# ZrrSkywalker/MonoDETR

Hardware: NVIDIA H100
Metric: images/sec (1280x384, fwd+bwd) (higher is better)
Workload: dtype f32 (BF16x3: error-compensated bf16 tensor-core products, fp32 accumulate)

## Files before the change

monodetr_b200/csrc/conv_gemm.cu:

```cuda
#include <cuda.h>
#include <cuda_runtime.h>
#include <stdint.h>
#include <stdlib.h>
#include <string.h>

#include "../../include/monodetr_b200.h"
#include "launch.cuh"
#include "tc_common.cuh"
#include "tma_host.cuh"

namespace {

using namespace mdb;

constexpr int BM = 128;
constexpr int BK = 32;
constexpr int kTileABytes = BM * 128;
constexpr int kChunkBytes = 32 * 128;
constexpr int kConsumerThreads = 256;
constexpr int kThreadsTC = kConsumerThreads + 128;
constexpr int kProducerRegs = 40;
constexpr int kConsumerRegs = 232;
constexpr int kMaxTaps = 9;

struct TcParams {
    int tiles_x, tiles_y, tw, th, tb;
    int Ho, Wo;
    int out_sy, out_sx, out_oy, out_ox, out_H, out_W;
    int in_sy, in_sx;
    int ntaps, cblocks;
    int tap_dy[kMaxTaps], tap_dx[kMaxTaps], tap_w[kMaxTaps];
    int rtiles_x, rtiles_y, rtw, rth, n_img, red_per_split;
    int kb_per_slice, slice_stride;
    int total_tiles, n_tiles_n, n_tiles_m;
    int w_sy, w_sx, wg_taps, wg_kw, wg_pad;
    int Mo_rows;
    int No, ldo;
    int relu, atomic_out, round_out;
    int epi_tma, epi_load, half_x, half_y, half_b;
    const float* bias;
    const float* residual;
    const float* relu_mask;
    const float* rowscale;
    float* out;
};

template <bool MN>
__device__ __forceinline__ uint32_t raw_off(int row, int k) {
    if constexpr (MN) return (uint32_t)((row >> 5) * kChunkBytes + k * 128 + (((((row & 31) >> 2) ^ (k & 7))) << 4) + (row & 3) * 4);
    else return (uint32_t)(row * 128 + (((k >> 2) ^ (row & 7)) << 4) + (k & 3) * 4);
}

__device__ __forceinline__ float trunc_tf32(float x) { return __uint_as_float(__float_as_uint(x) & 0xFFFFE000u); }

template <int BN, int STAGES, int MODE, int PREC>
struct TcSmem {
    static constexpr bool kConvB = !(PREC == 2 && MODE == 0);
    static constexpr int kRing = STAGES * (kTileABytes + BN * 128);
    static constexpr int kConvBuf = kConvB ? (PREC == 1 ? 2 : 1) * BN * 128 : 0;
    static constexpr int kConv = 2 * kConvBuf;
    static constexpr int kFixed = kRing + kConv + 1024  + 256 ;
    static constexpr int kChunks = BN / 32;
    static constexpr int kRoom = (227 * 1024 - kFixed) / (2 * 8192);
    static constexpr int kBufs = kRoom >= kChunks ? kChunks : BN < 256 ? 0 : kRoom >= 4 ? 4 : kRoom >= 2 ? 2 : kRoom;
    static constexpr int kStage = 2 * kBufs * 8192;
    static constexpr bool kTmaEpi = MODE == 0 && kBufs > 0;
    static constexpr int kBytes = kFixed + (kTmaEpi ? kStage : 0);
};

template <int BN, int STAGES, int MODE , bool B_MN, int PREC>
__global__ void __launch_bounds__(kThreadsTC, 1)
tc_conv_gemm_kernel(const __grid_constant__ CUtensorMap mapA, const __grid_constant__ CUtensorMap mapB,
                    const __grid_constant__ CUtensorMap mapO, const __grid_constant__ CUtensorMap mapR,
                    const __grid_constant__ TcParams p) {
    constexpr bool A_MN = (MODE == 1);
    static_assert(!(MODE == 1) || B_MN, "wgrad reads both operands MN-major");
    constexpr bool BF_B = (PREC == 2 && MODE == 0);
    static_assert(BN == 64 || BN == 128 || (BN == 256 && BF_B), "tile width");
    static_assert(!BF_B || !B_MN, "pre-split weights are K-major");
    constexpr bool CONVB = !BF_B;
    constexpr int kTileBBytes = BN * 128;
    constexpr int kRawBytes = kTileABytes + kTileBBytes;
    using SM = TcSmem<BN, STAGES, MODE, PREC>;
    constexpr int NACC = BN / 2;

    extern __shared__ __align__(1024) uint8_t smem[];
    uint8_t* stage_out = smem + STAGES * kRawBytes;
    uint8_t* bconv = stage_out + (SM::kTmaEpi ? SM::kStage : 0);
    uint64_t* full_bar = reinterpret_cast<uint64_t*>(bconv + SM::kConv);
    uint64_t* empty_bar = full_bar + STAGES;
    constexpr int kRound = SM::kBufs >= SM::kChunks ? SM::kChunks : 1;
    constexpr int kSlots = SM::kBufs / kRound > 0 ? SM::kBufs / kRound : 1;
    constexpr int kRounds = SM::kChunks / kRound;
    static_assert(kRounds % kSlots == 0, "every slot serves the same number of rounds per tile");
    uint64_t* epi_bar = empty_bar + STAGES;

    const int warp = threadIdx.x >> 5;
    const int lane = threadIdx.x & 31;

    struct Tile { int n0, img, y0, x0, m0, red_begin, iters, tap, slice; };
    auto decode = [&](int tix) {
        Tile t;
        t.n0 = (tix % p.n_tiles_n) * BN;
        int r = tix / p.n_tiles_n;
        t.img = t.y0 = t.x0 = t.m0 = t.red_begin = t.tap = t.slice = 0;
        if constexpr (MODE == 0) {
            const int per_img = p.tiles_x * p.tiles_y;
            t.iters = p.ntaps * p.cblocks;
            if (p.kb_per_slice > 0) {
                t.slice = r / p.n_tiles_m;
                r -= t.slice * p.n_tiles_m;
                t.red_begin = t.slice * p.kb_per_slice;
                t.iters = max(0, min(t.iters, t.red_begin + p.kb_per_slice) - t.red_begin);
            }
            const int grp = r / per_img;
            t.img = grp * p.tb;
            r -= grp * per_img;
            t.y0 = (r / p.tiles_x) * p.th;
            t.x0 = (r % p.tiles_x) * p.tw;
        } else {
            t.m0 = (r % p.n_tiles_m) * BM;
            r /= p.n_tiles_m;
            t.tap = r % p.wg_taps;
            const int z = r / p.wg_taps;
            const int total_red = p.n_img * p.rtiles_x * p.rtiles_y;
            t.red_begin = z * p.red_per_split;
            t.iters = max(0, min(total_red, t.red_begin + p.red_per_split) - t.red_begin);
        }
        return t;
    };

    if (threadIdx.x == 0) {
        if (smem_u32(smem) & 1023u) __trap();
        tma_prefetch_desc(&mapA);
        tma_prefetch_desc(&mapB);
        if (SM::kTmaEpi && p.epi_tma) {
            tma_prefetch_desc(&mapO);
            if (p.epi_load) tma_prefetch_desc(&mapR);
        }
        for (int s = 0; s < STAGES; ++s) {
            mbar_init(&full_bar[s], 1);
            mbar_init(&empty_bar[s], kConsumerThreads / 32);
        }
        for (int i = 0; i < 2 * kSlots; ++i) mbar_init(&epi_bar[i], 1);
        fence_mbar_init();
    }
    __syncthreads();
    asm volatile("griddepcontrol.wait;" ::: "memory");
    asm volatile("griddepcontrol.launch_dependents;" ::: "memory");

    if (warp >= kConsumerThreads / 32) {
        setmaxnreg_dec<kProducerRegs>();
        if (warp == kConsumerThreads / 32 && elect_one()) {
            int git = 0;
            for (int tix = blockIdx.x; tix < p.total_tiles; tix += gridDim.x) {
                const Tile t = decode(tix);
                for (int it = 0; it < t.iters; ++it, ++git) {
                    const int s = git % STAGES;
                    const uint32_t ph = (git / STAGES) & 1;
                    mbar_wait(&empty_bar[s], ph ^ 1);
                    uint8_t* a_dst = smem + s * kRawBytes;
                    uint8_t* b_dst = a_dst + kTileABytes;
                    mbar_arrive_expect_tx(&full_bar[s], kRawBytes);
                    if constexpr (MODE == 0) {
                        const int kit = t.red_begin + it;
                        const int tap = kit / p.cblocks;
                        const int cb = kit - tap * p.cblocks;
                        tma_load_4d(a_dst, &mapA, &full_bar[s], cb * BK, t.x0 * p.in_sx + p.tap_dx[tap],
                                    t.y0 * p.in_sy + p.tap_dy[tap], t.img);
                        if constexpr (BF_B) {
                            tma_load_3d(b_dst, &mapB, &full_bar[s], cb * 64, t.n0, p.tap_w[tap]);
                        } else if constexpr (!B_MN) {
                            tma_load_3d(b_dst, &mapB, &full_bar[s], cb * BK, t.n0, p.tap_w[tap]);
                        } else {
#pragma unroll
                            for (int j = 0; j < BN / 32; ++j)
                                tma_load_3d(b_dst + j * kChunkBytes, &mapB, &full_bar[s], t.n0 + j * 32, cb * BK, p.tap_w[tap]);
                        }
                    } else {
                        int r = t.red_begin + it;
                        const int per_img = p.rtiles_x * p.rtiles_y;
                        const int ri = r / per_img;
                        r -= ri * per_img;
                        const int ry = (r / p.rtiles_x) * p.rth;
                        const int rx = (r % p.rtiles_x) * p.rtw;
#pragma unroll
                        for (int j = 0; j < BM / 32; ++j)
                            tma_load_4d(a_dst + j * kChunkBytes, &mapA, &full_bar[s], t.m0 + j * 32, rx, ry, ri);
#pragma unroll
                        for (int j = 0; j < BN / 32; ++j)
                            tma_load_4d(b_dst + j * kChunkBytes, &mapB, &full_bar[s], t.n0 + j * 32,
                                        rx * p.w_sx + (t.tap % p.wg_kw) - p.wg_pad, ry * p.w_sy + (t.tap / p.wg_kw) - p.wg_pad, ri);
                    }
                }
            }
        }
        return;
    }

    setmaxnreg_inc<kConsumerRegs>();
    const int wg = warp >> 2;
    const int g = lane >> 2, tig = lane & 3;
    const int r0 = wg * 64 + (warp & 3) * 16 + g;
    const int ctid = threadIdx.x;
    const bool epi_tma = SM::kTmaEpi && p.epi_tma;
    const bool leader = (ctid & 127) == 0;
    uint8_t* my_stage = stage_out + wg * (SM::kStage / 2);
    uint64_t* my_epi_bar = epi_bar + wg * kSlots;
    uint32_t epi_use = 0;
    constexpr int KS = PREC == 2 ? 2 : 4;
    using Frag = uint32_t[KS][4];
    auto load_kblock = [&](int gi, int buf, Frag& hi, Frag& lo) {
        const int s = gi % STAGES;
        mbar_wait(&full_bar[s], (gi / STAGES) & 1);
        const uint8_t* a_raw = smem + s * kRawBytes;
        if constexpr (CONVB) {
            const uint8_t* b_raw = a_raw + kTileABytes;
            uint8_t* bc = bconv + buf * SM::kConvBuf;
            named_bar_sync(1, kConsumerThreads);
            if constexpr (PREC == 2) {
#pragma unroll
                for (int i = ctid; i < BN * 4; i += kConsumerThreads) {
                    const int n = i % BN, c = i / BN;
                    float x[8];
#pragma unroll
                    for (int e = 0; e < 8; ++e) x[e] = *reinterpret_cast<const float*>(b_raw + raw_off<B_MN>(n, 8 * c + e));
                    uint32_t hw[4], lw[4];
#pragma unroll
                    for (int e = 0; e < 4; ++e) {
                        const uint32_t h = pack_bf16x2(x[2 * e], x[2 * e + 1]);
                        hw[e] = h;
                        lw[e] = pack_bf16x2(x[2 * e] - __uint_as_float(h << 16), x[2 * e + 1] - __uint_as_float(h & 0xFFFF0000u));
                    }
                    uint8_t* brow = bc + n * 128;
                    *reinterpret_cast<uint4*>(brow + ((c ^ (n & 7)) << 4)) = make_uint4(hw[0], hw[1], hw[2], hw[3]);
                    *reinterpret_cast<uint4*>(brow + (((4 + c) ^ (n & 7)) << 4)) = make_uint4(lw[0], lw[1], lw[2], lw[3]);
                }
            } else {
#pragma unroll 4
                for (int i = ctid; i < BN * 8; i += kConsumerThreads) {
                    const int n = i % BN, c = i / BN;
                    float4 x;
                    if constexpr (B_MN) {
                        x.x = *reinterpret_cast<const float*>(b_raw + raw_off<true>(n, 4 * c));
                        x.y = *reinterpret_cast<const float*>(b_raw + raw_off<true>(n, 4 * c + 1));
                        x.z = *reinterpret_cast<const float*>(b_raw + raw_off<true>(n, 4 * c + 2));
                        x.w = *reinterpret_cast<const float*>(b_raw + raw_off<true>(n, 4 * c + 3));
                    } else {
                        x = *reinterpret_cast<const float4*>(b_raw + raw_off<false>(n, 4 * c));
                    }
                    const float4 h = make_float4(trunc_tf32(x.x), trunc_tf32(x.y), trunc_tf32(x.z), trunc_tf32(x.w));
                    const uint32_t off = n * 128 + ((c ^ (n & 7)) << 4);
                    *reinterpret_cast<float4*>(bc + off) = h;
                    if constexpr (PREC == 1)
                        *reinterpret_cast<float4*>(bc + kTileBBytes + off) = make_float4(x.x - h.x, x.y - h.y, x.z - h.z, x.w - h.w);
                }
            }
            fence_proxy_async_smem();
            named_bar_sync(1, kConsumerThreads);
        }
#pragma unroll
        for (int ks = 0; ks < KS; ++ks) {
#pragma unroll
            for (int f = 0; f < 4; ++f) {
                const int row = r0 + (f & 1) * 8;
                if constexpr (PREC == 2) {
                    const int k = ks * 16 + tig * 2 + (f >> 1) * 8;
                    float x0, x1;
                    if constexpr (A_MN) {
                        x0 = *reinterpret_cast<const float*>(a_raw + raw_off<true>(row, k));
                        x1 = *reinterpret_cast<const float*>(a_raw + raw_off<true>(row, k + 1));
                    } else {
                        const float2 v = *reinterpret_cast<const float2*>(a_raw + raw_off<false>(row, k));
                        x0 = v.x; x1 = v.y;
                    }
                    const uint32_t h = pack_bf16x2(x0, x1);
                    hi[ks][f] = h;
                    lo[ks][f] = pack_bf16x2(x0 - __uint_as_float(h << 16), x1 - __uint_as_float(h & 0xFFFF0000u));
                } else {
                    const int k = ks * 8 + tig + (f >> 1) * 4;
                    const float x = *reinterpret_cast<const float*>(a_raw + raw_off<A_MN>(row, k));
                    const float h = trunc_tf32(x);
                    hi[ks][f] = __float_as_uint(h);
                    lo[ks][f] = __float_as_uint(x - h);
                }
            }
        }
    };
    auto issue_kblock = [&](int gi, int buf, const Frag& hi, const Frag& lo, float (&acc)[NACC]) {
        const uint32_t b_addr = smem_u32(CONVB ? bconv + buf * SM::kConvBuf : smem + (gi % STAGES) * kRawBytes + kTileABytes);
        wgmma_fence();
#pragma unroll
        for (int ks = 0; ks < KS; ++ks) {
            const uint64_t bhi = make_wgmma_desc_sw128(b_addr + ks * 32);
            const uint64_t blo = make_wgmma_desc_sw128(b_addr + (PREC == 2 ? 64 : kTileBBytes) + ks * 32);
            if constexpr (PREC == 2) {
                if constexpr (BN == 256) {
                    wgmma_bf16_n256(acc, hi[ks], bhi, 1);
                    wgmma_bf16_n256(acc, lo[ks], bhi, 1);
                    wgmma_bf16_n256(acc, hi[ks], blo, 1);
                } else if constexpr (BN == 128) {
                    wgmma_bf16_n128(acc, hi[ks], bhi, 1);
                    wgmma_bf16_n128(acc, lo[ks], bhi, 1);
                    wgmma_bf16_n128(acc, hi[ks], blo, 1);
                } else {
                    wgmma_bf16_n64(acc, hi[ks], bhi, 1);
                    wgmma_bf16_n64(acc, lo[ks], bhi, 1);
                    wgmma_bf16_n64(acc, hi[ks], blo, 1);
                }
            } else {
                if constexpr (BN == 128) wgmma_tf32_n128(acc, hi[ks], bhi, 1);
                else wgmma_tf32_n64(acc, hi[ks], bhi, 1);
                if constexpr (PREC == 1) {
                    if constexpr (BN == 128) {
                        wgmma_tf32_n128(acc, lo[ks], bhi, 1);
                        wgmma_tf32_n128(acc, hi[ks], blo, 1);
                    } else {
                        wgmma_tf32_n64(acc, lo[ks], bhi, 1);
                        wgmma_tf32_n64(acc, hi[ks], blo, 1);
                    }
                }
            }
        }
        wgmma_commit();
    };
    int git = 0;
    for (int tix = blockIdx.x; tix < p.total_tiles; tix += gridDim.x) {
        const Tile t = decode(tix);
        if (p.atomic_out && t.iters == 0) continue;
        const int c1 = t.x0 + wg * p.half_x, c2 = t.y0 + wg * p.half_y, c3 = t.img + wg * p.half_b, c4 = t.slice;
        auto fetch_round = [&](int r) {
            uint8_t* dst = my_stage + (r % kSlots) * (kRound * 8192);
            mbar_arrive_expect_tx(&my_epi_bar[r % kSlots], kRound * 8192);
#pragma unroll
            for (int c = 0; c < kRound; ++c)
                tma_load_5d(dst + c * 8192, &mapR, &my_epi_bar[r % kSlots], t.n0 + 32 * (r * kRound + c), c1, c2, c3, c4);
        };
        if (epi_tma && p.epi_load && leader) {
            bulk_wait_read_all();
#pragma unroll
            for (int r = 0; r < kSlots; ++r) fetch_round(r);
        }
        float acc[NACC];
#pragma unroll
        for (int i = 0; i < NACC; ++i) acc[i] = 0.f;
        if (t.iters > 0) {
            Frag ahi0, alo0, ahi1, alo1;
            auto step = [&](int it, const Frag& chi, const Frag& clo, Frag& nhi, Frag& nlo) {
                issue_kblock(git + it, it & 1, chi, clo, acc);
                wgmma_wait<1>();
                wgmma_fence_operands(nhi);
                wgmma_fence_operands(nlo);
                if (it > 0) {
                    __syncwarp();
                    if (lane == 0) mbar_arrive(&empty_bar[(git + it - 1) % STAGES]);
                }
                if (it + 1 < t.iters) load_kblock(git + it + 1, (it + 1) & 1, nhi, nlo);
            };
            load_kblock(git, 0, ahi0, alo0);
            for (int it = 0; it < t.iters; it += 2) {
                step(it, ahi0, alo0, ahi1, alo1);
                if (it + 1 < t.iters) step(it + 1, ahi1, alo1, ahi0, alo0);
            }
            wgmma_wait<0>();
            wgmma_fence_operands(acc);
            wgmma_fence_operands(ahi0);
            wgmma_fence_operands(alo0);
            wgmma_fence_operands(ahi1);
            wgmma_fence_operands(alo1);
            __syncwarp();
            if (lane == 0) mbar_arrive(&empty_bar[(git + t.iters - 1) % STAGES]);
            git += t.iters;
        }

        if (epi_tma) {
            if (p.bias) {
#pragma unroll
                for (int j = 0; j < BN / 8; ++j) {
                    const int n = t.n0 + j * 8 + tig * 2;
                    if (n >= p.No) continue;
                    const float b0 = p.bias[n], b1 = p.bias[n + 1];
                    acc[4 * j] += b0; acc[4 * j + 1] += b1; acc[4 * j + 2] += b0; acc[4 * j + 3] += b1;
                }
            }
            constexpr int kMB = 8 < kRound * 4 ? 8 : kRound * 4;
#pragma unroll
            for (int r = 0; r < kRounds; ++r) {
                uint8_t* slot = my_stage + (r % kSlots) * (kRound * 8192);
                if (p.epi_load) {
                    mbar_wait(&my_epi_bar[r % kSlots], (epi_use + r / kSlots) & 1);
                } else {
                    if (leader) bulk_wait_read<kSlots - 1>();
                    named_bar_sync_diverged(2 + wg, 128);
                }
#pragma unroll
                for (int h = 0; h < 2; ++h) {
                    const int row = r0 + h * 8, rr = row - 64 * wg;
                    const float* gmask = nullptr;
                    if (p.relu_mask && p.epi_load != 2) {
                        const int lyt = row / p.tw, lx = row - lyt * p.tw;
                        const int ib = lyt / p.th, ly = lyt - ib * p.th;
                        const int y = t.y0 + ly, x = t.x0 + lx, img = t.img + ib;
                        if ((y < p.Ho) && (x < p.Wo) && (img < p.n_img))
                            gmask = p.relu_mask + (size_t)((img * p.out_H + y * p.out_sy + p.out_oy) * p.out_W + x * p.out_sx + p.out_ox) * p.ldo;
                    }
#pragma unroll
                    for (int j0 = 0; j0 < kRound * 4; j0 += kMB) {
                        float2 mv[kMB];
#pragma unroll
                        for (int u = 0; u < kMB; ++u) {
                            const int n = t.n0 + (r * kRound * 4 + j0 + u) * 8 + tig * 2;
                            mv[u] = (gmask && n < p.No) ? *reinterpret_cast<const float2*>(gmask + n) : make_float2(0.f, 0.f);
                        }
#pragma unroll
                        for (int u = 0; u < kMB; ++u) {
                            const int jl = j0 + u, j = r * kRound * 4 + jl, n = t.n0 + j * 8 + tig * 2;
                            if (n >= p.No) continue;
                            float2* sp = reinterpret_cast<float2*>(slot + (jl >> 2) * 8192 + raw_off<false>(rr, (j & 3) * 8 + tig * 2));
                            float v[2] = {acc[4 * j + 2 * h], acc[4 * j + 2 * h + 1]};
                            if (p.epi_load == 1) { const float2 e = *sp; v[0] += e.x; v[1] += e.y; }
                            if (p.relu) { v[0] = fmaxf(v[0], 0.f); v[1] = fmaxf(v[1], 0.f); }
                            if (p.relu_mask) {
                                const float2 m = p.epi_load == 2 ? *sp : mv[u];
                                v[0] = m.x > 0.f ? v[0] : 0.f; v[1] = m.y > 0.f ? v[1] : 0.f;
                            }
                            if (p.round_out) { v[0] = round_tf32(v[0]); v[1] = round_tf32(v[1]); }
                            *sp = make_float2(v[0], v[1]);
                        }
                    }
                }
                fence_proxy_async_smem();
                named_bar_sync_diverged(2 + wg, 128);
                if (leader) {
#pragma unroll
                    for (int c = 0; c < kRound; ++c)
                        tma_store_5d(&mapO, slot + c * 8192, t.n0 + 32 * (r * kRound + c), c1, c2, c3, c4);
                    bulk_commit();
                    if (p.epi_load && r + kSlots < kRounds) {
                        bulk_wait_read_all();
                        fetch_round(r + kSlots);
                    }
                }
                __syncwarp();
            }
            epi_use += kRounds / kSlots;
            continue;
        }
#pragma unroll
        for (int h = 0; h < 2; ++h) {
            const int row = r0 + h * 8;
            bool ok;
            size_t roff;
            float rsc = 1.f;
            if constexpr (MODE == 0) {
                const int lyt = row / p.tw, lx = row - lyt * p.tw;
                const int ib = lyt / p.th, ly = lyt - ib * p.th;
                const int y = t.y0 + ly, x = t.x0 + lx, img = t.img + ib;
                ok = (y < p.Ho) && (x < p.Wo) && (img < p.n_img);
                const int oy = y * p.out_sy + p.out_oy, ox = x * p.out_sx + p.out_ox;
                roff = (size_t)((img * p.out_H + oy) * p.out_W + ox) * p.ldo + (size_t)t.slice * p.slice_stride;
            } else {
                ok = (t.m0 + row) < p.Mo_rows;
                if (ok && p.rowscale) rsc = p.rowscale[t.m0 + row];
                roff = (size_t)(t.tap * p.Mo_rows + t.m0 + row) * p.ldo;
            }
            if (!ok) continue;
            const bool vec = !(p.ldo & 1);
#pragma unroll
            for (int j = 0; j < BN / 8; ++j) {
                const int n = t.n0 + j * 8 + tig * 2;
                if (n >= p.No) continue;
                float v[2] = {acc[4 * j + 2 * h] * rsc, acc[4 * j + 2 * h + 1] * rsc};
                const bool pair = vec && n + 1 < p.No;
                if (p.bias) { v[0] += p.bias[n]; if (pair) v[1] += p.bias[n + 1]; }
                if (p.residual) {
                    if (pair) { const float2 e = *reinterpret_cast<const float2*>(p.residual + roff + n); v[0] += e.x; v[1] += e.y; }
                    else v[0] += p.residual[roff + n];
                }
                if (p.relu) { v[0] = fmaxf(v[0], 0.f); v[1] = fmaxf(v[1], 0.f); }
                if (p.relu_mask) {
                    if (pair) {
                        const float2 m = *reinterpret_cast<const float2*>(p.relu_mask + roff + n);
                        v[0] = m.x > 0.f ? v[0] : 0.f; v[1] = m.y > 0.f ? v[1] : 0.f;
                    } else {
                        v[0] = p.relu_mask[roff + n] > 0.f ? v[0] : 0.f;
                    }
                }
                if (p.round_out) { v[0] = round_tf32(v[0]); v[1] = round_tf32(v[1]); }
                float* dst = p.out + roff + n;
                if (pair) {
                    if (p.atomic_out) red_add_v2_f32(dst, v[0], v[1]);
                    else *reinterpret_cast<float2*>(dst) = make_float2(v[0], v[1]);
                } else {
                    for (int e = 0; e < 2 && n + e < p.No; ++e) {
                        float x = e == 0 ? v[0] : acc[4 * j + 2 * h + 1] * rsc;
                        if (e == 1) {
                            if (p.bias) x += p.bias[n + 1];
                            if (p.residual) x += p.residual[roff + n + 1];
                            if (p.relu) x = fmaxf(x, 0.f);
                            if (p.relu_mask) x = p.relu_mask[roff + n + 1] > 0.f ? x : 0.f;
                            if (p.round_out) x = round_tf32(x);
                        }
                        if (p.atomic_out) atomicAdd(dst + e, x);
                        else dst[e] = x;
                    }
                }
            }
        }
    }
    if (epi_tma && leader) bulk_wait_all();
}

int g_precision = 2;

constexpr int kMaxDevices = 64;
struct DeviceState {
    float* ws = nullptr;
    size_t ws_bytes = 0;
};
DeviceState g_dev[kMaxDevices];

int current_device() {
    int dev = 0;
    if (cudaGetDevice(&dev) != cudaSuccess || dev < 0 || dev >= kMaxDevices) return 0;
    return dev;
}

template <int BN, int STAGES, int MODE, bool B_MN, int PREC>
int launch_tc(const CUtensorMap& a, const CUtensorMap& b, const CUtensorMap& o, const CUtensorMap& r, TcParams p, dim3 grid,
              cudaStream_t stream) {
    constexpr int smem = TcSmem<BN, STAGES, MODE, PREC>::kBytes;
    static_assert(smem <= 227 * 1024, "dynamic shared memory budget");
    if (!TcSmem<BN, STAGES, MODE, PREC>::kTmaEpi) p.epi_tma = p.epi_load = 0;
    auto kern = tc_conv_gemm_kernel<BN, STAGES, MODE, B_MN, PREC>;
    const cudaError_t e = set_max_dynamic_smem(kern, smem);
    if (e != cudaSuccess) return (int)e;
    p.n_tiles_n = (int)grid.x;
    p.n_tiles_m = (int)grid.y;
    p.total_tiles = (int)(grid.x * grid.y * grid.z);
    int ctas = num_sms();
    if (ctas > p.total_tiles) ctas = p.total_tiles;
    if (ctas < 1) return 0;
    static const bool pdl = getenv("MDB_NO_PDL") == nullptr;
    if (pdl) {
        cudaLaunchConfig_t cfg;
        memset(&cfg, 0, sizeof(cfg));
        cfg.gridDim = dim3((unsigned)ctas, 1, 1);
        cfg.blockDim = dim3((unsigned)kThreadsTC, 1, 1);
        cfg.dynamicSmemBytes = smem;
        cfg.stream = stream;
        cudaLaunchAttribute attr[1];
        attr[0].id = cudaLaunchAttributeProgrammaticStreamSerialization;
        attr[0].val.programmaticStreamSerializationAllowed = 1;
        cfg.attrs = attr;
        cfg.numAttrs = 1;
        return (int)cudaLaunchKernelEx(&cfg, kern, a, b, o, r, p);
    }
    kern<<<ctas, kThreadsTC, smem, stream>>>(a, b, o, r, p);
    return (int)cudaGetLastError();
}

__global__ void splitk_reduce_kernel(const float4* __restrict__ ws, const float4* __restrict__ bias, float4* __restrict__ y,
                                     long long n4, int N4, int slices, long long stride4) {
    for (long long i = blockIdx.x * (long long)blockDim.x + threadIdx.x; i < n4; i += (long long)gridDim.x * blockDim.x) {
        float4 a = bias ? bias[i % N4] : make_float4(0.f, 0.f, 0.f, 0.f);
        for (int z = 0; z < slices; ++z) {
            const float4 v = ws[z * stride4 + i];
            a.x += v.x; a.y += v.y; a.z += v.z; a.w += v.w;
        }
        y[i] = a;
    }
}

int splitk_workspace(size_t bytes, float** out) {
    DeviceState& d = g_dev[current_device()];
    if (bytes > d.ws_bytes || !d.ws) return MDB_EWORKSPACE;
    *out = d.ws;
    return 0;
}

void pick_tile(int W, int H, int n_pix, int* tw, int* th) {
    int best_tw = n_pix, best_waste = 1 << 30;
    for (int w = n_pix; w >= 1; w >>= 1) {
        const int h = n_pix / w;
        const int tx = (W + w - 1) / w, ty = (H + h - 1) / h;
        const int waste = tx * w * ty * h - W * H;
        if (waste < best_waste) { best_waste = waste; best_tw = w; }
    }
    *tw = best_tw;
    *th = n_pix / best_tw;
}

void pick_tile3(int W, int H, int B, int n_pix, int* tw, int* th, int* tb) {
    long long best = -1;
    *tw = n_pix; *th = 1; *tb = 1;
    for (int b = 1; b <= n_pix; b <<= 1)
        for (int w = n_pix / b; w >= 1; w >>= 1) {
            const int h = n_pix / b / w;
            if (b > 1 && b >= 2 * B) continue;
// ... 452 lines not shown
```

monodetr_b200/csrc/tc_common.cuh:

```cuda
#pragma once
#include <cuda.h>
#include <cuda_runtime.h>
#include <stdint.h>

namespace mdb {

__device__ __forceinline__ uint32_t smem_u32(const void* p) {
    return static_cast<uint32_t>(__cvta_generic_to_shared(p));
}

__device__ __forceinline__ bool elect_one() {
    uint32_t pred = 0;
    asm volatile(
        "{\n\t.reg .b32 rx;\n\t.reg .pred px;\n\t"
        "elect.sync rx|px, 0xffffffff;\n\t"
        "selp.b32 %0, 1, 0, px;\n\t}"
        : "=r"(pred));
    return pred != 0;
}

__device__ __forceinline__ void mbar_init(uint64_t* bar, uint32_t count) {
    asm volatile("mbarrier.init.shared::cta.b64 [%0], %1;" ::"r"(smem_u32(bar)), "r"(count) : "memory");
}
__device__ __forceinline__ void fence_mbar_init() {
    asm volatile("fence.mbarrier_init.release.cluster;" ::: "memory");
}
__device__ __forceinline__ void mbar_arrive_expect_tx(uint64_t* bar, uint32_t bytes) {
    asm volatile("mbarrier.arrive.expect_tx.shared::cta.b64 _, [%0], %1;" ::"r"(smem_u32(bar)), "r"(bytes) : "memory");
}
__device__ __forceinline__ void mbar_arrive(uint64_t* bar) {
    asm volatile("mbarrier.arrive.shared::cta.b64 _, [%0];" ::"r"(smem_u32(bar)) : "memory");
}
__device__ __forceinline__ bool mbar_try_wait(uint64_t* bar, uint32_t parity) {
    uint32_t ok;
    asm volatile(
        "{\n\t.reg .pred p;\n\t"
        "mbarrier.try_wait.parity.shared::cta.b64 p, [%1], %2;\n\t"
        "selp.b32 %0, 1, 0, p;\n\t}"
        : "=r"(ok)
        : "r"(smem_u32(bar)), "r"(parity)
        : "memory");
    return ok != 0;
}
static __device__ __noinline__ void mbar_slow_path(uint64_t& t0) {
    uint64_t t;
    asm volatile("mov.u64 %0, %globaltimer;" : "=l"(t));
    if (t0 == 0) t0 = t;
    else if (t - t0 > 2000000000ull) __trap();
}
__device__ __forceinline__ void mbar_wait(uint64_t* bar, uint32_t parity) {
    uint32_t spins = 0;
    uint64_t t0 = 0;
    while (!mbar_try_wait(bar, parity)) {
        if (++spins == 16384u) {
            spins = 0;
            mbar_slow_path(t0);
        }
    }
}

__device__ __forceinline__ void fence_proxy_async_smem() { asm volatile("fence.proxy.async.shared::cta;" ::: "memory"); }
__device__ __forceinline__ void named_bar_sync(int id, int count) { asm volatile("bar.sync %0, %1;" ::"r"(id), "r"(count) : "memory"); }
__device__ __forceinline__ void named_bar_sync_diverged(int id, int count) {
    asm volatile("barrier.sync %0, %1;" ::"r"(id), "r"(count) : "memory");
}

__device__ __forceinline__ void tma_prefetch_desc(const CUtensorMap* m) {
    asm volatile("prefetch.tensormap [%0];" ::"l"(reinterpret_cast<uint64_t>(m)) : "memory");
}
__device__ __forceinline__ void tma_load_2d(void* dst, const CUtensorMap* m, uint64_t* bar, int c0, int c1) {
    asm volatile(
        "cp.async.bulk.tensor.2d.shared::cluster.global.mbarrier::complete_tx::bytes [%0], [%1, {%3, %4}], [%2];" ::"r"(
            smem_u32(dst)),
        "l"(reinterpret_cast<uint64_t>(m)), "r"(smem_u32(bar)), "r"(c0), "r"(c1)
        : "memory");
}
__device__ __forceinline__ void tma_load_3d(void* dst, const CUtensorMap* m, uint64_t* bar, int c0, int c1, int c2) {
    asm volatile(
        "cp.async.bulk.tensor.3d.shared::cluster.global.mbarrier::complete_tx::bytes [%0], [%1, {%3, %4, %5}], [%2];" ::"r"(
            smem_u32(dst)),
        "l"(reinterpret_cast<uint64_t>(m)), "r"(smem_u32(bar)), "r"(c0), "r"(c1), "r"(c2)
        : "memory");
}
__device__ __forceinline__ void tma_load_4d(void* dst, const CUtensorMap* m, uint64_t* bar, int c0, int c1, int c2,
                                            int c3) {
    asm volatile(
        "cp.async.bulk.tensor.4d.shared::cluster.global.mbarrier::complete_tx::bytes [%0], [%1, {%3, %4, %5, %6}], "
        "[%2];" ::"r"(smem_u32(dst)),
        "l"(reinterpret_cast<uint64_t>(m)), "r"(smem_u32(bar)), "r"(c0), "r"(c1), "r"(c2), "r"(c3)
        : "memory");
}
__device__ __forceinline__ void tma_load_5d(void* dst, const CUtensorMap* m, uint64_t* bar, int c0, int c1, int c2,
                                            int c3, int c4) {
    asm volatile(
        "cp.async.bulk.tensor.5d.shared::cluster.global.mbarrier::complete_tx::bytes [%0], [%1, {%3, %4, %5, %6, %7}], "
        "[%2];" ::"r"(smem_u32(dst)),
        "l"(reinterpret_cast<uint64_t>(m)), "r"(smem_u32(bar)), "r"(c0), "r"(c1), "r"(c2), "r"(c3), "r"(c4)
        : "memory");
}
__device__ __forceinline__ void tma_store_5d(const CUtensorMap* m, const void* src, int c0, int c1, int c2, int c3, int c4) {
    asm volatile("cp.async.bulk.tensor.5d.global.shared::cta.bulk_group [%0, {%2, %3, %4, %5, %6}], [%1];"
                 ::"l"(reinterpret_cast<uint64_t>(m)), "r"(smem_u32(src)), "r"(c0), "r"(c1), "r"(c2), "r"(c3), "r"(c4)
                 : "memory");
}
__device__ __forceinline__ void bulk_commit() { asm volatile("cp.async.bulk.commit_group;" ::: "memory"); }
__device__ __forceinline__ void bulk_wait_read_all() { asm volatile("cp.async.bulk.wait_group.read 0;" ::: "memory"); }
template <int N>
__device__ __forceinline__ void bulk_wait_read() { asm volatile("cp.async.bulk.wait_group.read %0;" ::"n"(N) : "memory"); }
__device__ __forceinline__ void bulk_wait_all() { asm volatile("cp.async.bulk.wait_group 0;" ::: "memory"); }

template <int N>
__device__ __forceinline__ void setmaxnreg_dec() { asm volatile("setmaxnreg.dec.sync.aligned.u32 %0;" ::"n"(N)); }
template <int N>
__device__ __forceinline__ void setmaxnreg_inc() { asm volatile("setmaxnreg.inc.sync.aligned.u32 %0;" ::"n"(N)); }

__device__ __forceinline__ void wgmma_fence() { asm volatile("wgmma.fence.sync.aligned;" ::: "memory"); }
__device__ __forceinline__ void wgmma_commit() { asm volatile("wgmma.commit_group.sync.aligned;" ::: "memory"); }
__device__ __forceinline__ void wgmma_wait_all() { asm volatile("wgmma.wait_group.sync.aligned 0;" ::: "memory"); }
template <int N>
__device__ __forceinline__ void wgmma_wait() { asm volatile("wgmma.wait_group.sync.aligned %0;" ::"n"(N) : "memory"); }
template <int N>
__device__ __forceinline__ void wgmma_fence_operands(float (&d)[N]) {
#pragma unroll
    for (int i = 0; i < N; ++i) asm volatile("" : "+f"(d[i])::"memory");
}
template <int M, int N>
__device__ __forceinline__ void wgmma_fence_operands(uint32_t (&a)[M][N]) {
#pragma unroll
    for (int i = 0; i < M; ++i)
#pragma unroll
        for (int j = 0; j < N; ++j) asm volatile("" : "+r"(a[i][j])::"memory");
}
__device__ __forceinline__ void wgmma_bf16_n64(float (&d)[32], const uint32_t (&a)[4], uint64_t bdesc, int scale_d) {
    asm volatile(
        "{\n\t.reg .pred p;\n\t"
        "setp.ne.b32 p, %37, 0;\n\t"
        "wgmma.mma_async.sync.aligned.m64n64k16.f32.bf16.bf16 "
        "{%0, %1, %2, %3, %4, %5, %6, %7, %8, %9, %10, %11, %12, %13, %14, %15, "
        "%16, %17, %18, %19, %20, %21, %22, %23, %24, %25, %26, %27, %28, %29, %30, %31"
        "}, {%32, %33, %34, %35}, %36, p, 1, 1, 0;\n\t}"
        : "+f"(d[0]), "+f"(d[1]), "+f"(d[2]), "+f"(d[3]), "+f"(d[4]), "+f"(d[5]), "+f"(d[6]), "+f"(d[7]), "+f"(d[8]), "+f"(d[9]), "+f"(d[10]), "+f"(d[11]), "+f"(d[12]), "+f"(d[13]), "+f"(d[14]), "+f"(d[15]), "+f"(d[16]), "+f"(d[17]), "+f"(d[18]), "+f"(d[19]), "+f"(d[20]), "+f"(d[21]), "+f"(d[22]), "+f"(d[23]), "+f"(d[24]), "+f"(d[25]), "+f"(d[26]), "+f"(d[27]), "+f"(d[28]), "+f"(d[29]), "+f"(d[30]), "+f"(d[31])
        : "r"(a[0]), "r"(a[1]), "r"(a[2]), "r"(a[3]), "l"(bdesc), "r"(scale_d));
}
__device__ __forceinline__ void wgmma_bf16_n128(float (&d)[64], const uint32_t (&a)[4], uint64_t bdesc, int scale_d) {
    asm volatile(
        "{\n\t.reg .pred p;\n\t"
        "setp.ne.b32 p, %69, 0;\n\t"
        "wgmma.mma_async.sync.aligned.m64n128k16.f32.bf16.bf16 "
        "{%0, %1, %2, %3, %4, %5, %6, %7, %8, %9, %10, %11, %12, %13, %14, %15, "
        "%16, %17, %18, %19, %20, %21, %22, %23, %24, %25, %26, %27, %28, %29, %30, %31, "
        "%32, %33, %34, %35, %36, %37, %38, %39, %40, %41, %42, %43, %44, %45, %46, %47, "
        "%48, %49, %50, %51, %52, %53, %54, %55, %56, %57, %58, %59, %60, %61, %62, %63"
        "}, {%64, %65, %66, %67}, %68, p, 1, 1, 0;\n\t}"
        : "+f"(d[0]), "+f"(d[1]), "+f"(d[2]), "+f"(d[3]), "+f"(d[4]), "+f"(d[5]), "+f"(d[6]), "+f"(d[7]), "+f"(d[8]), "+f"(d[9]), "+f"(d[10]), "+f"(d[11]), "+f"(d[12]), "+f"(d[13]), "+f"(d[14]), "+f"(d[15]), "+f"(d[16]), "+f"(d[17]), "+f"(d[18]), "+f"(d[19]), "+f"(d[20]), "+f"(d[21]), "+f"(d[22]), "+f"(d[23]), "+f"(d[24]), "+f"(d[25]), "+f"(d[26]), "+f"(d[27]), "+f"(d[28]), "+f"(d[29]), "+f"(d[30]), "+f"(d[31]), "+f"(d[32]), "+f"(d[33]), "+f"(d[34]), "+f"(d[35]), "+f"(d[36]), "+f"(d[37]), "+f"(d[38]), "+f"(d[39]), "+f"(d[40]), "+f"(d[41]), "+f"(d[42]), "+f"(d[43]), "+f"(d[44]), "+f"(d[45]), "+f"(d[46]), "+f"(d[47]), "+f"(d[48]), "+f"(d[49]), "+f"(d[50]), "+f"(d[51]), "+f"(d[52]), "+f"(d[53]), "+f"(d[54]), "+f"(d[55]), "+f"(d[56]), "+f"(d[57]), "+f"(d[58]), "+f"(d[59]), "+f"(d[60]), "+f"(d[61]), "+f"(d[62]), "+f"(d[63])
        : "r"(a[0]), "r"(a[1]), "r"(a[2]), "r"(a[3]), "l"(bdesc), "r"(scale_d));
}
__device__ __forceinline__ void wgmma_bf16_n256(float (&d)[128], const uint32_t (&a)[4], uint64_t bdesc, int scale_d) {
    asm volatile(
        "{\n\t.reg .pred p;\n\t"
        "setp.ne.b32 p, %133, 0;\n\t"
        "wgmma.mma_async.sync.aligned.m64n256k16.f32.bf16.bf16 "
        "{"
        "%0, %1, %2, %3, %4, %5, %6, %7, %8, %9, %10, %11, %12, %13, %14, %15, "
        "%16, %17, %18, %19, %20, %21, %22, %23, %24, %25, %26, %27, %28, %29, %30, %31, "
        "%32, %33, %34, %35, %36, %37, %38, %39, %40, %41, %42, %43, %44, %45, %46, %47, "
        "%48, %49, %50, %51, %52, %53, %54, %55, %56, %57, %58, %59, %60, %61, %62, %63, "
        "%64, %65, %66, %67, %68, %69, %70, %71, %72, %73, %74, %75, %76, %77, %78, %79, "
        "%80, %81, %82, %83, %84, %85, %86, %87, %88, %89, %90, %91, %92, %93, %94, %95, "
        "%96, %97, %98, %99, %100, %101, %102, %103, %104, %105, %106, %107, %108, %109, %110, %111, "
        "%112, %113, %114, %115, %116, %117, %118, %119, %120, %121, %122, %123, %124, %125, %126, %127"
        "}, {%128, %129, %130, %131}, %132, p, 1, 1, 0;\n\t}"
        : "+f"(d[0]), "+f"(d[1]), "+f"(d[2]), "+f"(d[3]), "+f"(d[4]), "+f"(d[5]), "+f"(d[6]), "+f"(d[7]), "+f"(d[8]), "+f"(d[9]), "+f"(d[10]), "+f"(d[11]), "+f"(d[12]), "+f"(d[13]), "+f"(d[14]), "+f"(d[15]), "+f"(d[16]), "+f"(d[17]), "+f"(d[18]), "+f"(d[19]), "+f"(d[20]), "+f"(d[21]), "+f"(d[22]), "+f"(d[23]), "+f"(d[24]), "+f"(d[25]), "+f"(d[26]), "+f"(d[27]), "+f"(d[28]), "+f"(d[29]), "+f"(d[30]), "+f"(d[31]), "+f"(d[32]), "+f"(d[33]), "+f"(d[34]), "+f"(d[35]), "+f"(d[36]), "+f"(d[37]), "+f"(d[38]), "+f"(d[39]), "+f"(d[40]), "+f"(d[41]), "+f"(d[42]), "+f"(d[43]), "+f"(d[44]), "+f"(d[45]), "+f"(d[46]), "+f"(d[47]), "+f"(d[48]), "+f"(d[49]), "+f"(d[50]), "+f"(d[51]), "+f"(d[52]), "+f"(d[53]), "+f"(d[54]), "+f"(d[55]), "+f"(d[56]), "+f"(d[57]), "+f"(d[58]), "+f"(d[59]), "+f"(d[60]), "+f"(d[61]), "+f"(d[62]), "+f"(d[63]), "+f"(d[64]), "+f"(d[65]), "+f"(d[66]), "+f"(d[67]), "+f"(d[68]), "+f"(d[69]), "+f"(d[70]), "+f"(d[71]), "+f"(d[72]), "+f"(d[73]), "+f"(d[74]), "+f"(d[75]), "+f"(d[76]), "+f"(d[77]), "+f"(d[78]), "+f"(d[79]), "+f"(d[80]), "+f"(d[81]), "+f"(d[82]), "+f"(d[83]), "+f"(d[84]), "+f"(d[85]), "+f"(d[86]), "+f"(d[87]), "+f"(d[88]), "+f"(d[89]), "+f"(d[90]), "+f"(d[91]), "+f"(d[92]), "+f"(d[93]), "+f"(d[94]), "+f"(d[95]), "+f"(d[96]), "+f"(d[97]), "+f"(d[98]), "+f"(d[99]), "+f"(d[100]), "+f"(d[101]), "+f"(d[102]), "+f"(d[103]), "+f"(d[104]), "+f"(d[105]), "+f"(d[106]), "+f"(d[107]), "+f"(d[108]), "+f"(d[109]), "+f"(d[110]), "+f"(d[111]), "+f"(d[112]), "+f"(d[113]), "+f"(d[114]), "+f"(d[115]), "+f"(d[116]), "+f"(d[117]), "+f"(d[118]), "+f"(d[119]), "+f"(d[120]), "+f"(d[121]), "+f"(d[122]), "+f"(d[123]), "+f"(d[124]), "+f"(d[125]), "+f"(d[126]), "+f"(d[127])
        : "r"(a[0]), "r"(a[1]), "r"(a[2]), "r"(a[3]), "l"(bdesc), "r"(scale_d));
}
__device__ __forceinline__ void wgmma_tf32_n16(float (&d)[8], const uint32_t (&a)[4], uint64_t bdesc, int scale_d) {
    asm volatile(
        "{\n\t.reg .pred p;\n\t"
        "setp.ne.b32 p, %13, 0;\n\t"
        "wgmma.mma_async.sync.aligned.m64n16k8.f32.tf32.tf32 "
        "{%0, %1, %2, %3, %4, %5, %6, %7"
        "}, {%8, %9, %10, %11}, %12, p, 1, 1;\n\t}"
        : "+f"(d[0]), "+f"(d[1]), "+f"(d[2]), "+f"(d[3]), "+f"(d[4]), "+f"(d[5]), "+f"(d[6]), "+f"(d[7])
        : "r"(a[0]), "r"(a[1]), "r"(a[2]), "r"(a[3]), "l"(bdesc), "r"(scale_d));
}
__device__ __forceinline__ void wgmma_tf32_n32(float (&d)[16], const uint32_t (&a)[4], uint64_t bdesc, int scale_d) {
    asm volatile(
        "{\n\t.reg .pred p;\n\t"
        "setp.ne.b32 p, %21, 0;\n\t"
        "wgmma.mma_async.sync.aligned.m64n32k8.f32.tf32.tf32 "
        "{%0, %1, %2, %3, %4, %5, %6, %7, %8, %9, %10, %11, %12, %13, %14, %15"
        "}, {%16, %17, %18, %19}, %20, p, 1, 1;\n\t}"
        : "+f"(d[0]), "+f"(d[1]), "+f"(d[2]), "+f"(d[3]), "+f"(d[4]), "+f"(d[5]), "+f"(d[6]), "+f"(d[7]), "+f"(d[8]), "+f"(d[9]), "+f"(d[10]), "+f"(d[11]), "+f"(d[12]), "+f"(d[13]), "+f"(d[14]), "+f"(d[15])
        : "r"(a[0]), "r"(a[1]), "r"(a[2]), "r"(a[3]), "l"(bdesc), "r"(scale_d));
}

__device__ __forceinline__ void wgmma_tf32_n64(float (&d)[32], const uint32_t (&a)[4], uint64_t bdesc, int scale_d) {
    asm volatile(
        "{\n\t.reg .pred p;\n\t"
        "setp.ne.b32 p, %37, 0;\n\t"
        "wgmma.mma_async.sync.aligned.m64n64k8.f32.tf32.tf32 "
        "{%0, %1, %2, %3, %4, %5, %6, %7, %8, %9, %10, %11, %12, %13, %14, %15, "
        "%16, %17, %18, %19, %20, %21, %22, %23, %24, %25, %26, %27, %28, %29, %30, %31"
        "}, {%32, %33, %34, %35}, %36, p, 1, 1;\n\t}"
        : "+f"(d[0]), "+f"(d[1]), "+f"(d[2]), "+f"(d[3]), "+f"(d[4]), "+f"(d[5]), "+f"(d[6]), "+f"(d[7]), "+f"(d[8]), "+f"(d[9]), "+f"(d[10]), "+f"(d[11]), "+f"(d[12]), "+f"(d[13]), "+f"(d[14]), "+f"(d[15]), "+f"(d[16]), "+f"(d[17]), "+f"(d[18]), "+f"(d[19]), "+f"(d[20]), "+f"(d[21]), "+f"(d[22]), "+f"(d[23]), "+f"(d[24]), "+f"(d[25]), "+f"(d[26]), "+f"(d[27]), "+f"(d[28]), "+f"(d[29]), "+f"(d[30]), "+f"(d[31])
        : "r"(a[0]), "r"(a[1]), "r"(a[2]), "r"(a[3]), "l"(bdesc), "r"(scale_d));
}
__device__ __forceinline__ void wgmma_tf32_n128(float (&d)[64], const uint32_t (&a)[4], uint64_t bdesc, int scale_d) {
    asm volatile(
        "{\n\t.reg .pred p;\n\t"
        "setp.ne.b32 p, %69, 0;\n\t"
        "wgmma.mma_async.sync.aligned.m64n128k8.f32.tf32.tf32 "
        "{%0, %1, %2, %3, %4, %5, %6, %7, %8, %9, %10, %11, %12, %13, %14, %15, "
        "%16, %17, %18, %19, %20, %21, %22, %23, %24, %25, %26, %27, %28, %29, %30, %31, "
        "%32, %33, %34, %35, %36, %37, %38, %39, %40, %41, %42, %43, %44, %45, %46, %47, "
        "%48, %49, %50, %51, %52, %53, %54, %55, %56, %57, %58, %59, %60, %61, %62, %63"
        "}, {%64, %65, %66, %67}, %68, p, 1, 1;\n\t}"
        : "+f"(d[0]), "+f"(d[1]), "+f"(d[2]), "+f"(d[3]), "+f"(d[4]), "+f"(d[5]), "+f"(d[6]), "+f"(d[7]), "+f"(d[8]), "+f"(d[9]), "+f"(d[10]), "+f"(d[11]), "+f"(d[12]), "+f"(d[13]), "+f"(d[14]), "+f"(d[15]), "+f"(d[16]), "+f"(d[17]), "+f"(d[18]), "+f"(d[19]), "+f"(d[20]), "+f"(d[21]), "+f"(d[22]), "+f"(d[23]), "+f"(d[24]), "+f"(d[25]), "+f"(d[26]), "+f"(d[27]), "+f"(d[28]), "+f"(d[29]), "+f"(d[30]), "+f"(d[31]), "+f"(d[32]), "+f"(d[33]), "+f"(d[34]), "+f"(d[35]), "+f"(d[36]), "+f"(d[37]), "+f"(d[38]), "+f"(d[39]), "+f"(d[40]), "+f"(d[41]), "+f"(d[42]), "+f"(d[43]), "+f"(d[44]), "+f"(d[45]), "+f"(d[46]), "+f"(d[47]), "+f"(d[48]), "+f"(d[49]), "+f"(d[50]), "+f"(d[51]), "+f"(d[52]), "+f"(d[53]), "+f"(d[54]), "+f"(d[55]), "+f"(d[56]), "+f"(d[57]), "+f"(d[58]), "+f"(d[59]), "+f"(d[60]), "+f"(d[61]), "+f"(d[62]), "+f"(d[63])
        : "r"(a[0]), "r"(a[1]), "r"(a[2]), "r"(a[3]), "l"(bdesc), "r"(scale_d));
}


__device__ __forceinline__ uint32_t pack_bf16x2(float lo, float hi) {
    uint32_t r;
    asm("cvt.rn.bf16x2.f32 %0, %1, %2;" : "=r"(r) : "f"(hi), "f"(lo));
    return r;
}

__device__ __forceinline__ uint64_t make_wgmma_desc_sw128(uint32_t smem_addr) {
    return (uint64_t)((smem_addr & 0x3FFFFu) >> 4) | ((uint64_t)1 << 16) | ((uint64_t)(1024 >> 4) << 32) | ((uint64_t)1 << 62);
}

__device__ __forceinline__ float round_tf32(float v) {
    uint32_t r;
    asm("cvt.rna.tf32.f32 %0, %1;" : "=r"(r) : "f"(v));
    return __uint_as_float(r);
}

__device__ __forceinline__ void red_add_v4_f32(float* addr, float a, float b, float c, float d) {
    asm volatile("red.global.add.v4.f32 [%0], {%1, %2, %3, %4};" ::"l"(addr), "f"(a), "f"(b), "f"(c), "f"(d) : "memory");
}

__device__ __forceinline__ void red_add_v2_f32(float* addr, float a, float b) {
    asm volatile("red.global.add.v2.f32 [%0], {%1, %2};" ::"l"(addr), "f"(a), "f"(b) : "memory");
}

}
```

Before: 173.2.

## Offload wgrad B-operand bf16 split to dedicated converter warps with ring buffer

```diff
diff --git a/monodetr_b200/csrc/conv_gemm.cu b/monodetr_b200/csrc/conv_gemm.cu
--- a/monodetr_b200/csrc/conv_gemm.cu
+++ b/monodetr_b200/csrc/conv_gemm.cu
@@ -56,9 +56,11 @@
 template <int BN, int STAGES, int MODE, int PREC>
 struct TcSmem {
     static constexpr bool kConvB = !(PREC == 2 && MODE == 0);
+    static constexpr bool kConvRing = PREC == 2 && MODE == 1;
     static constexpr int kRing = STAGES * (kTileABytes + BN * 128);
     static constexpr int kConvBuf = kConvB ? (PREC == 1 ? 2 : 1) * BN * 128 : 0;
-    static constexpr int kConv = 2 * kConvBuf;
+    static constexpr int kConvSets = kConvRing ? 4 : 2;
+    static constexpr int kConv = kConvSets * kConvBuf;
     static constexpr int kFixed = kRing + kConv + 1024  + 256 ;
     static constexpr int kChunks = BN / 32;
     static constexpr int kRoom = (227 * 1024 - kFixed) / (2 * 8192);
@@ -79,6 +81,11 @@
     static_assert(BN == 64 || BN == 128 || (BN == 256 && BF_B), "tile width");
     static_assert(!BF_B || !B_MN, "pre-split weights are K-major");
     constexpr bool CONVB = !BF_B;
+    constexpr bool CONV_RING = TcSmem<BN, STAGES, MODE, PREC>::kConvRing;
+    static_assert(!CONV_RING || BN == 128, "the converters' item mapping and the transposed wgmma are written for BN = 128");
+    constexpr int kConvWarps = 3;
+    constexpr int kConvSets = TcSmem<BN, STAGES, MODE, PREC>::kConvSets;
+    constexpr int kPlaneBytes = BN * 32 * 2;
     constexpr int kTileBBytes = BN * 128;
     constexpr int kRawBytes = kTileABytes + kTileBBytes;
     using SM = TcSmem<BN, STAGES, MODE, PREC>;
@@ -94,6 +101,9 @@
     constexpr int kRounds = SM::kChunks / kRound;
     static_assert(kRounds % kSlots == 0, "every slot serves the same number of rounds per tile");
     uint64_t* epi_bar = empty_bar + STAGES;
+    uint64_t* conv_full = epi_bar + 2 * kSlots;
+    uint64_t* conv_empty = conv_full + kConvSets;
+    static_assert(2 * STAGES + 2 * kSlots + 2 * kConvSets <= 32, "barriers fit their 256 bytes");
 
     const int warp = threadIdx.x >> 5;
     const int lane = threadIdx.x & 31;
@@ -140,9 +150,15 @@
         }
         for (int s = 0; s < STAGES; ++s) {
             mbar_init(&full_bar[s], 1);
-            mbar_init(&empty_bar[s], kConsumerThreads / 32);
+            mbar_init(&empty_bar[s], kConsumerThreads / 32 + (CONV_RING ? kConvWarps : 0));
         }
         for (int i = 0; i < 2 * kSlots; ++i) mbar_init(&epi_bar[i], 1);
+        if constexpr (CONV_RING) {
+            for (int c = 0; c < kConvSets; ++c) {
+                mbar_init(&conv_full[c], kConvWarps);
+                mbar_init(&conv_empty[c], kConsumerThreads / 32);
+            }
+        }
         fence_mbar_init();
     }
     __syncthreads();
@@ -195,6 +211,45 @@
                 }
             }
         }
+        if constexpr (CONV_RING) {
+            if (warp > kConsumerThreads / 32) {
+                const int ct = threadIdx.x - kConsumerThreads - 32;
+                int git = 0;
+                for (int tix = blockIdx.x; tix < p.total_tiles; tix += gridDim.x) {
+                    const Tile t = decode(tix);
+                    for (int it = 0; it < t.iters; ++it, ++git) {
+                        const int s = git % STAGES, c = git % kConvSets;
+                        mbar_wait(&conv_empty[c], ((git / kConvSets) & 1) ^ 1);
+                        mbar_wait(&full_bar[s], (git / STAGES) & 1);
+                        const uint8_t* b_raw = smem + s * kRawBytes + kTileABytes;
+                        uint8_t* bc = bconv + c * SM::kConvBuf;
+                        for (int i = ct; i < BN * 4; i += 32 * kConvWarps) {
+                            const int kl = i & 7, grp = (i >> 3) % (BN / 8), k = (i >> 3) / (BN / 8) * 8 + kl;
+                            const uint8_t* src = b_raw + (grp >> 2) * kChunkBytes + k * 128;
+                            const float4 v0 = *reinterpret_cast<const float4*>(src + (((2 * (grp & 3)) ^ kl) << 4));
+                            const float4 v1 = *reinterpret_cast<const float4*>(src + (((2 * (grp & 3) + 1) ^ kl) << 4));
+                            const float x[8] = {v0.x, v0.y, v0.z, v0.w, v1.x, v1.y, v1.z, v1.w};
+                            uint32_t hw[4], lw[4];
+#pragma unroll
+                            for (int e = 0; e < 4; ++e) {
+                                const uint32_t h = pack_bf16x2(x[2 * e], x[2 * e + 1]);
+                                hw[e] = h;
+                                lw[e] = pack_bf16x2(x[2 * e] - __uint_as_float(h << 16), x[2 * e + 1] - __uint_as_float(h & 0xFFFF0000u));
+                            }
+                            uint8_t* dst = bc + (grp >> 3) * 4096 + (k >> 3) * 1024 + kl * 128 + (((grp & 7) ^ kl) << 4);
+                            *reinterpret_cast<uint4*>(dst) = make_uint4(hw[0], hw[1], hw[2], hw[3]);
+                            *reinterpret_cast<uint4*>(dst + kPlaneBytes) = make_uint4(lw[0], lw[1], lw[2], lw[3]);
+                        }
+                        fence_proxy_async_smem();
+                        __syncwarp();
+                        if (lane == 0) {
+                            mbar_arrive(&conv_full[c]);
+                            mbar_arrive(&empty_bar[s]);
+                        }
+                    }
+                }
+            }
+        }
         return;
     }
 
@@ -214,7 +269,7 @@
         const int s = gi % STAGES;
         mbar_wait(&full_bar[s], (gi / STAGES) & 1);
         const uint8_t* a_raw = smem + s * kRawBytes;
-        if constexpr (CONVB) {
+        if constexpr (CONVB && !CONV_RING) {
             const uint8_t* b_raw = a_raw + kTileABytes;
             uint8_t* bc = bconv + buf * SM::kConvBuf;
             named_bar_sync(1, kConsumerThreads);
@@ -286,8 +341,27 @@
                 }
             }
         }
+        if constexpr (CONV_RING) {
+            __syncwarp();
+            if (lane == 0) mbar_arrive(&empty_bar[s]);
+        }
     };
     auto issue_kblock = [&](int gi, int buf, const Frag& hi, const Frag& lo, float (&acc)[NACC]) {
+        if constexpr (CONV_RING) {
+            mbar_wait(&conv_full[gi % kConvSets], (gi / kConvSets) & 1);
+            const uint32_t b_addr = smem_u32(bconv + (gi % kConvSets) * SM::kConvBuf);
+            wgmma_fence();
+#pragma unroll
+            for (int ks = 0; ks < KS; ++ks) {
+                const uint64_t bhi = make_wgmma_desc_sw128_mn(b_addr + ks * 2048, 4096, 1024);
+                const uint64_t blo = make_wgmma_desc_sw128_mn(b_addr + kPlaneBytes + ks * 2048, 4096, 1024);
+                wgmma_bf16_n128<1>(acc, hi[ks], bhi, 1);
+                wgmma_bf16_n128<1>(acc, lo[ks], bhi, 1);
+                wgmma_bf16_n128<1>(acc, hi[ks], blo, 1);
+            }
+            wgmma_commit();
+            return;
+        }
         const uint32_t b_addr = smem_u32(CONVB ? bconv + buf * SM::kConvBuf : smem + (gi % STAGES) * kRawBytes + kTileABytes);
         wgmma_fence();
 #pragma unroll
@@ -353,7 +427,10 @@
                 wgmma_fence_operands(nlo);
                 if (it > 0) {
                     __syncwarp();
-                    if (lane == 0) mbar_arrive(&empty_bar[(git + it - 1) % STAGES]);
+                    if (lane == 0) {
+                        if constexpr (CONV_RING) mbar_arrive(&conv_empty[(git + it - 1) % kConvSets]);
+                        else mbar_arrive(&empty_bar[(git + it - 1) % STAGES]);
+                    }
                 }
                 if (it + 1 < t.iters) load_kblock(git + it + 1, (it + 1) & 1, nhi, nlo);
             };
@@ -369,7 +446,10 @@
             wgmma_fence_operands(ahi1);
             wgmma_fence_operands(alo1);
             __syncwarp();
-            if (lane == 0) mbar_arrive(&empty_bar[(git + t.iters - 1) % STAGES]);
+            if (lane == 0) {
+                if constexpr (CONV_RING) mbar_arrive(&conv_empty[(git + t.iters - 1) % kConvSets]);
+                else mbar_arrive(&empty_bar[(git + t.iters - 1) % STAGES]);
+            }
             git += t.iters;
         }
 
@@ -445,6 +525,26 @@
             }
             epi_use += kRounds / kSlots;
             continue;
+        }
+        if constexpr (CONV_RING) {
+            if ((reinterpret_cast<uintptr_t>(p.out) & 15u) == 0) {
+                const bool odd = tig & 1;
+                const int row = r0 + (odd ? 8 : 0);
+                const bool ok = t.m0 + row < p.Mo_rows;
+                const float rsc = (ok && p.rowscale) ? p.rowscale[t.m0 + row] : 1.f;
+                float* dst = p.out + (size_t)(t.tap * p.Mo_rows + t.m0 + row) * p.ldo;
+#pragma unroll
+                for (int j = 0; j < BN / 8; ++j) {
+                    const float k0 = odd ? acc[4 * j + 2] : acc[4 * j], k1 = odd ? acc[4 * j + 3] : acc[4 * j + 1];
+                    const float r0v = __shfl_xor_sync(0xffffffffu, odd ? acc[4 * j] : acc[4 * j + 2], 1);
+                    const float r1v = __shfl_xor_sync(0xffffffffu, odd ? acc[4 * j + 1] : acc[4 * j + 3], 1);
+                    const int n = t.n0 + j * 8 + (tig & 2) * 2;
+                    if (!ok || n >= p.No) continue;
+                    if (odd) red_add_v4_f32(dst + n, r0v * rsc, r1v * rsc, k0 * rsc, k1 * rsc);
+                    else red_add_v4_f32(dst + n, k0 * rsc, k1 * rsc, r0v * rsc, r1v * rsc);
+                }
+                continue;
+            }
         }
 #pragma unroll
         for (int h = 0; h < 2; ++h) {
diff --git a/monodetr_b200/csrc/tc_common.cuh b/monodetr_b200/csrc/tc_common.cuh
--- a/monodetr_b200/csrc/tc_common.cuh
+++ b/monodetr_b200/csrc/tc_common.cuh
@@ -142,6 +142,7 @@
         : "+f"(d[0]), "+f"(d[1]), "+f"(d[2]), "+f"(d[3]), "+f"(d[4]), "+f"(d[5]), "+f"(d[6]), "+f"(d[7]), "+f"(d[8]), "+f"(d[9]), "+f"(d[10]), "+f"(d[11]), "+f"(d[12]), "+f"(d[13]), "+f"(d[14]), "+f"(d[15]), "+f"(d[16]), "+f"(d[17]), "+f"(d[18]), "+f"(d[19]), "+f"(d[20]), "+f"(d[21]), "+f"(d[22]), "+f"(d[23]), "+f"(d[24]), "+f"(d[25]), "+f"(d[26]), "+f"(d[27]), "+f"(d[28]), "+f"(d[29]), "+f"(d[30]), "+f"(d[31])
         : "r"(a[0]), "r"(a[1]), "r"(a[2]), "r"(a[3]), "l"(bdesc), "r"(scale_d));
 }
+template <int TRANS_B = 0>
 __device__ __forceinline__ void wgmma_bf16_n128(float (&d)[64], const uint32_t (&a)[4], uint64_t bdesc, int scale_d) {
     asm volatile(
         "{\n\t.reg .pred p;\n\t"
@@ -151,9 +152,9 @@
         "%16, %17, %18, %19, %20, %21, %22, %23, %24, %25, %26, %27, %28, %29, %30, %31, "
         "%32, %33, %34, %35, %36, %37, %38, %39, %40, %41, %42, %43, %44, %45, %46, %47, "
         "%48, %49, %50, %51, %52, %53, %54, %55, %56, %57, %58, %59, %60, %61, %62, %63"
-        "}, {%64, %65, %66, %67}, %68, p, 1, 1, 0;\n\t}"
+        "}, {%64, %65, %66, %67}, %68, p, 1, 1, %70;\n\t}"
         : "+f"(d[0]), "+f"(d[1]), "+f"(d[2]), "+f"(d[3]), "+f"(d[4]), "+f"(d[5]), "+f"(d[6]), "+f"(d[7]), "+f"(d[8]), "+f"(d[9]), "+f"(d[10]), "+f"(d[11]), "+f"(d[12]), "+f"(d[13]), "+f"(d[14]), "+f"(d[15]), "+f"(d[16]), "+f"(d[17]), "+f"(d[18]), "+f"(d[19]), "+f"(d[20]), "+f"(d[21]), "+f"(d[22]), "+f"(d[23]), "+f"(d[24]), "+f"(d[25]), "+f"(d[26]), "+f"(d[27]), "+f"(d[28]), "+f"(d[29]), "+f"(d[30]), "+f"(d[31]), "+f"(d[32]), "+f"(d[33]), "+f"(d[34]), "+f"(d[35]), "+f"(d[36]), "+f"(d[37]), "+f"(d[38]), "+f"(d[39]), "+f"(d[40]), "+f"(d[41]), "+f"(d[42]), "+f"(d[43]), "+f"(d[44]), "+f"(d[45]), "+f"(d[46]), "+f"(d[47]), "+f"(d[48]), "+f"(d[49]), "+f"(d[50]), "+f"(d[51]), "+f"(d[52]), "+f"(d[53]), "+f"(d[54]), "+f"(d[55]), "+f"(d[56]), "+f"(d[57]), "+f"(d[58]), "+f"(d[59]), "+f"(d[60]), "+f"(d[61]), "+f"(d[62]), "+f"(d[63])
-        : "r"(a[0]), "r"(a[1]), "r"(a[2]), "r"(a[3]), "l"(bdesc), "r"(scale_d));
+        : "r"(a[0]), "r"(a[1]), "r"(a[2]), "r"(a[3]), "l"(bdesc), "r"(scale_d), "n"(TRANS_B));
 }
 __device__ __forceinline__ void wgmma_bf16_n256(float (&d)[128], const uint32_t (&a)[4], uint64_t bdesc, int scale_d) {
     asm volatile(
@@ -229,6 +230,10 @@
 __device__ __forceinline__ uint64_t make_wgmma_desc_sw128(uint32_t smem_addr) {
     return (uint64_t)((smem_addr & 0x3FFFFu) >> 4) | ((uint64_t)1 << 16) | ((uint64_t)(1024 >> 4) << 32) | ((uint64_t)1 << 62);
 }
+__device__ __forceinline__ uint64_t make_wgmma_desc_sw128_mn(uint32_t smem_addr, uint32_t lbo, uint32_t sbo) {
+    return (uint64_t)((smem_addr & 0x3FFFFu) >> 4) | ((uint64_t)((lbo >> 4) & 0x3FFFu) << 16) |
+           ((uint64_t)((sbo >> 4) & 0x3FFFu) << 32) | ((uint64_t)1 << 62);
+}
 
 __device__ __forceinline__ float round_tf32(float v) {
     uint32_t r;
```

New measurement: 177.0 (median of 6 runs). 2.2% higher.
